# ZhuoQiuMcgill/ReinforcementLearning4MeshGeneration

Measured on AMD Instinct MI355X. Metric: env-steps/sec at N_envs=4096 per GPU, boundary() domain, 1 MI355X, higher is better.
Workload: dtype f64

## Files before the change

reinforcementlearning4meshgeneration_amd/build.py:

```python
from __future__ import annotations

import os
import shutil
import subprocess
import sys

PKG_DIR = os.path.dirname(os.path.abspath(__file__))
CSRC = os.path.join(PKG_DIR, "csrc")
LIB_NAME = "libmeshenv_hip.so"
LIB_PATH = os.path.join(PKG_DIR, LIB_NAME)
SOURCES = ["meshenv_hip.hip"]
ARCH = "gfx950"
PUBLIC_HEADERS = ["meshenv.h", "meshenv_optim.h", "meshenv_td3_actor_grad.h", "meshenv_ppo_grad.h", "meshenv_rollout.h"]

HIPCC_FLAGS = ["-O3", "-std=c++17", "-ffp-contract=off", "-fhip-fp32-correctly-rounded-divide-sqrt",
               "-fno-fast-math", "-fPIC", "-shared", f"--offload-arch={ARCH}", "-Wall", "-Wno-unused-function",
               "-mllvm", "-disable-machine-licm", "-mllvm", "-amdgpu-atomic-optimizer-strategy=None"]


def hipcc_path() -> str:
    for cand in (os.environ.get("HIPCC"), shutil.which("hipcc"), "/opt/rocm/bin/hipcc"):
        if cand and os.path.exists(cand):
            return cand
    raise RuntimeError("hipcc not found (need ROCm to build libmeshenv_hip.so)")


def needs_build() -> bool:
    if not os.path.exists(LIB_PATH):
        return True
    t = os.path.getmtime(LIB_PATH)
    deps = [os.path.join(CSRC, f) for f in sorted(os.listdir(CSRC)) if f.endswith((".h", ".hip"))]
    deps += [os.path.join(os.path.dirname(PKG_DIR), "include", h) for h in PUBLIC_HEADERS]
    return any(os.path.getmtime(d) > t for d in deps)


def build(force: bool = False, verbose: bool = False, extra_flags=()) -> str:
    if not force and not needs_build():
        return LIB_PATH
    cmd = [hipcc_path(), *HIPCC_FLAGS, *extra_flags, "-o", LIB_PATH] + [os.path.join(CSRC, s) for s in SOURCES]
    if verbose:
        print(" ".join(cmd), flush=True)
    subprocess.check_call(cmd, cwd=CSRC)
    import hashlib
    import json
    h = hashlib.sha256()
    root = os.path.dirname(PKG_DIR)
    files = sorted(os.path.join(CSRC, f) for f in os.listdir(CSRC) if f.endswith((".h", ".hip"))) + [os.path.join(root, "include", h) for h in PUBLIC_HEADERS]
    for f in files:
        h.update(os.path.relpath(f, root).encode())
        h.update(open(f, "rb").read())
# ... 7 lines not shown
```

reinforcementlearning4meshgeneration_amd/csrc/meshenv_fused.h:

```cpp
#pragma once

#include "meshenv_actor.h"
#include "meshenv_kernels.h"

namespace meshenv {

struct GroupActorArgs {
    GroupArgs g;
    ActorWeights W;
    float *actions_next;
    float *eps_out;
    unsigned long long seed, counter;
    int sample;
    int pad;
};

__host__ __device__ __forceinline__ size_t group_actor_lds_bytes(int cap)
{
    return group_lds_bytes(cap, 16) + sizeof(float) * kActorLdsFloats;
}

template <bool kDefaultParams, bool kSmall = false>
__global__ void __launch_bounds__(64 * 16)
k_step_group_actor(GroupActorArgs A)
{
    extern __shared__ double2 smem[];
    float *lds = (float *)((char *)smem + group_lds_bytes(A.g.cap, 16));
    step_group_body<16, kDefaultParams, false, kSmall>(A.g, lds);
    ActorHead hd;
    actor_request_weights(hd, A.W, threadIdx.x, true);
    __syncthreads();
    actor_forward_tile(A.W, hd, A.g.S.n_envs, blockIdx.x * kActEnvs, nullptr, nullptr, A.actions_next, A.sample, A.seed, A.counter,
                       A.eps_out, lds, threadIdx.x, 64 * 16);
}

}
```

reinforcementlearning4meshgeneration_amd/csrc/meshenv_hip.hip:

```cpp
#include "../../include/meshenv.h"
#include "../../include/meshenv_optim.h"
#include "../../include/meshenv_td3_actor_grad.h"
#include "../../include/meshenv_ppo_grad.h"
#include "../../include/meshenv_rollout.h"

#include <hip/hip_runtime.h>
#include <link.h>

#include <cmath>
#include <cstdio>
#include <cstdlib>
#include <cstring>
#include <mutex>
#include <string>
#include <vector>

#include "meshenv_actor.h"
#include "meshenv_domgen.h"
#include "meshenv_kernels.h"
#include "meshenv_quality.h"
#include "meshenv_smooth.h"
#include "meshenv_samples.h"
#include "meshenv_fused.h"
#include "meshenv_policy.h"
// ... 403 lines not shown
    constexpr int kLdsCap = 160 * 1024;
    if (lds > 64 * 1024) {
        CREATE_HIP(hipFuncSetAttribute((const void *)k_step<false, false>, hipFuncAttributeMaxDynamicSharedMemorySize, kLdsCap));
        CREATE_HIP(hipFuncSetAttribute((const void *)k_step<true, false>, hipFuncAttributeMaxDynamicSharedMemorySize, kLdsCap));
        CREATE_HIP(hipFuncSetAttribute((const void *)k_step<false, true>, hipFuncAttributeMaxDynamicSharedMemorySize, kLdsCap));
        CREATE_HIP(hipFuncSetAttribute((const void *)k_step<true, true>, hipFuncAttributeMaxDynamicSharedMemorySize, kLdsCap));
        CREATE_HIP(hipFuncSetAttribute((const void *)k_step<false, false, true>, hipFuncAttributeMaxDynamicSharedMemorySize, kLdsCap));
        CREATE_HIP(hipFuncSetAttribute((const void *)k_step<true, false, true>, hipFuncAttributeMaxDynamicSharedMemorySize, kLdsCap));
        CREATE_HIP(hipFuncSetAttribute((const void *)k_step<false, true, true>, hipFuncAttributeMaxDynamicSharedMemorySize, kLdsCap));
        CREATE_HIP(hipFuncSetAttribute((const void *)k_step<true, true, true>, hipFuncAttributeMaxDynamicSharedMemorySize, kLdsCap));
        CREATE_HIP(hipFuncSetAttribute((const void *)k_step<false, true, false, false, true>, hipFuncAttributeMaxDynamicSharedMemorySize, kLdsCap));
        CREATE_HIP(hipFuncSetAttribute((const void *)k_reset, hipFuncAttributeMaxDynamicSharedMemorySize, kLdsCap));
        CREATE_HIP(hipFuncSetAttribute((const void *)k_init_domains, hipFuncAttributeMaxDynamicSharedMemorySize, kLdsCap));
    }
    CREATE_HIP(upload_atan_state());

    {
        int n_cu = 256;
        CREATE_HIP(hipDeviceGetAttribute(&n_cu, hipDeviceAttributeMultiprocessorCount, device));
        if (n_cu <= 0) n_cu = 256;
        h->n_cu = n_cu;
        int G = 1;
        const char *force = getenv("MESHENV_GROUP");
        int want = 1;
        if (force) want = atoi(force);
        else if (n_envs <= n_cu * 16) {
            int g = 1;
            while (g * 2 <= n_envs / n_cu && g * 2 <= 16) g *= 2;
            want = g >= 8 ? g : 1;
        }
        for (int g : {16, 8})
            if (g <= want && group_lds_bytes(cap, g) <= 150 * 1024) { G = g; break; }
        if (!force && (G < 8 || n_envs > n_cu * G)) G = 1;
        if (G == 1 && want == 16 && n_envs <= n_cu * 16 && group_lds_bytes(cap, 16) > 150 * 1024) {
            std::vector<int2> pack((size_t)n_envs);
            size_t worst = 0;
            for (int w0 = 0; w0 < n_envs; w0 += 16) {
                size_t off = 0;
                for (int e = w0; e < w0 + 16 && e < n_envs; e++) {
                    const int d = env_domain_host[e];
                    const int n0 = dom_offsets_host[d + 1] - dom_offsets_host[d];
                    const int cap_e = (n0 + 15) / 16 * 16;
                    pack[(size_t)e] = make_int2((int)off, cap_e);
                    off += lds_bytes_for(cap_e);
                }
                worst = off > worst ? off : worst;
            }
            worst = (worst + 31) / 32 * 32;
            if (worst + 16 * sizeof(Handoff) <= (size_t)kLdsCap) {
                G = 16;
                h->env_lds_host.swap(pack);
                h->ho_off = (int)worst;
            }
        }
        MeshEnvParams def;
        meshenv_default_params(&def);
        h->default_params = prm.radius == def.radius && prm.max_ref_angle == def.max_ref_angle && prm.key_lambda == def.key_lambda &&
                            prm.min_degree == def.min_degree && prm.max_degree == def.max_degree &&
                            prm.same_point_eps == def.same_point_eps && prm.ray_length == def.ray_length;
        if (!h->default_params) G = 1;
        if (!h->default_params) h->env_lds_host.clear();
        h->group = G;
        h->group_lds = h->env_lds_host.empty() ? group_lds_bytes(cap, G) : (size_t)h->ho_off + 16 * sizeof(Handoff);
        {
            const char *lz = getenv("MESHENV_LAZY");
            const bool lazy = lz ? atoi(lz) != 0 : n_envs >= 8192;
            const char *lt = getenv("MESHENV_LIGHT");
// ... 718 lines not shown
    }
    return MESHENV_OK;
}

static int launch_step(MeshEnv *h, int n_steps, const float *actions_dev, float *obs_dev, double *reward_dev,
                       uint8_t *done_dev, uint8_t *complete_dev, float *terminal_obs_dev, int auto_reset)
{
    if (!h) return MESHENV_E_ARG;
    if (!actions_dev || !obs_dev || !reward_dev || !done_dev || !complete_dev) return fail_arg(h, "meshenv_step: null device pointer");
    if (n_steps <= 0) return fail_arg(h, "meshenv_rollout: n_steps must be positive");
    if (n_steps > 1 && h->reselect_pending) {
        h->err = "meshenv_rollout: the first step after meshenv_smooth must be a meshenv_step (it commits the re-selection "
                 "the candidate rebuild parked, include/meshenv.h)";
        return MESHENV_E_STATE;
    }
    MESHENV_ON_DEVICE(h);
    const size_t slot = (size_t)(h->ev_count % MESHENV_TIMING_POOL);
    const long long pos = h->timing > 0 ? (h->launch_count++ % (2LL * h->timing)) : -1;
    if (pos == 0) HIP_TRY(h, hipEventRecord(h->ev[2 * slot], h->stream));
    if (n_steps == 1 && h->group > 1 && !h->front_moved) {
        const int G = h->group;
        const dim3 grid((h->n_envs + G - 1) / G), block(64 * G);
        GroupArgs A;
        A.S = h->S;
        A.outs.obs_out = obs_dev; A.outs.reward = reward_dev; A.outs.done = done_dev; A.outs.complete = complete_dev;
        A.outs.term_obs = terminal_obs_dev;
        A.actions = actions_dev;
        A.step0 = (unsigned long long)h->steps_done;
        A.cap = h->cap;
        A.auto_reset = auto_reset;
        A.env_lds = h->env_lds;
        A.ho_off = h->ho_off;
        A.pad = 0;
        if (h->env_lds) hipLaunchKernelGGL((k_step_group<16, true, true>), grid, block, h->group_lds, h->stream, A);
        else if (h->cap <= 64 && G == 16) hipLaunchKernelGGL((k_step_group<16, true, false, true>), grid, block, h->group_lds, h->stream, A);
        else if (h->cap <= 64) hipLaunchKernelGGL((k_step_group<8, true, false, true>), grid, block, h->group_lds, h->stream, A);
        else if (G == 16) hipLaunchKernelGGL((k_step_group<16, true>), grid, block, h->group_lds, h->stream, A);
        else hipLaunchKernelGGL((k_step_group<8, true>), grid, block, h->group_lds, h->stream, A);
    } else {
        const dim3 grid(h->n_envs), block(64);
#define MESHENV_LAUNCH_STEP(MULTI, DEF)                                                                                      \
    do {                                                                                                                     \
        KStepArgs ka;                                                                                                        \
        ka.S = h->S; ka.cap = h->cap; ka.n_steps = n_steps; ka.actions = actions_dev; ka.obs_out = obs_dev;                  \
        ka.reward = reward_dev; ka.done = done_dev; ka.complete = complete_dev; ka.term_obs = terminal_obs_dev;              \
        ka.auto_reset = auto_reset; ka.step0 = (unsigned long long)h->steps_done;                                            \
        if (h->front_moved) hipLaunchKernelGGL((k_step<MULTI, DEF, true>), grid, block, h->lds, h->stream, ka);              \
        else if (DEF && !MULTI && (h->stage_bits & 2) && h->cap <= 64)                                                       \
            hipLaunchKernelGGL((k_step<false, DEF, false, DEF, DEF>), grid, block, h->lds, h->stream, ka);                   \
        else if (DEF && !MULTI && (h->stage_bits & 2))                                                                       \
            hipLaunchKernelGGL((k_step<false, DEF, false, false, DEF>), grid, block, h->lds, h->stream, ka);                 \
        else if (DEF && h->cap <= 64) hipLaunchKernelGGL((k_step<MULTI, DEF, false, DEF>), grid, block, h->lds, h->stream, ka); \
        else hipLaunchKernelGGL((k_step<MULTI, DEF>), grid, block, h->lds, h->stream, ka);                                   \
    } while (0)
        if (n_steps == 1) {
            auto_reset = (auto_reset ? 1 : 0) | h->stage_bits;
            if (h->default_params) MESHENV_LAUNCH_STEP(false, true);
            else MESHENV_LAUNCH_STEP(false, false);
        } else {
            if (h->default_params) MESHENV_LAUNCH_STEP(true, true);
            else MESHENV_LAUNCH_STEP(true, false);
        }
#undef MESHENV_LAUNCH_STEP
    }
    HIP_TRY(h, hipGetLastError());
    if (h->reselect_pending) {
        hipLaunchKernelGGL(k_apply_reselect, dim3(h->n_envs), dim3(64), 0, h->stream, h->S, h->pend, h->pend_obs, obs_dev);
        HIP_TRY(h, hipGetLastError());
        h->reselect_pending = false;
    }
    h->steps_done += (uint64_t)n_steps;
// ... 482 lines not shown
        h->err = "meshenv_step_actor: env and actor must be on the same device and stream (meshenv_set_stream / meshenv_actor_set_stream)";
        return MESHENV_E_STATE;
    }
    const bool fusable = h->group == 16 && h->default_params && !h->front_moved && !h->env_lds &&
                         h->timing == 0 && !h->reselect_pending && group_actor_lds_bytes(h->cap) <= 160 * 1024;
    if (!fusable) {
        const int rc = launch_step(h, 1, actions_dev, obs_dev, reward_dev, done_dev, complete_dev, terminal_obs_dev, auto_reset);
        if (rc != MESHENV_OK) return rc;
        const int ra = actor_launch(a, "meshenv_step_actor", h->n_envs, obs_dev, nullptr, actions_next_dev, sample, seed, counter,
                                    eps_out_dev);
        if (ra != MESHENV_OK) h->err = a->err;
        return ra;
    }
    MESHENV_ON_DEVICE(h);
    if (!h->fused_ready) {
        HIP_TRY(h, hipFuncSetAttribute((const void *)k_step_group_actor<true>, hipFuncAttributeMaxDynamicSharedMemorySize, 160 * 1024));
        HIP_TRY(h, hipFuncSetAttribute((const void *)k_step_group_actor<true, true>, hipFuncAttributeMaxDynamicSharedMemorySize, 160 * 1024));
        h->fused_ready = true;
    }
    GroupActorArgs GA;
    GA.g.S = h->S;
    GA.g.outs.obs_out = obs_dev; GA.g.outs.reward = reward_dev; GA.g.outs.done = done_dev; GA.g.outs.complete = complete_dev;
    GA.g.outs.term_obs = terminal_obs_dev;
    GA.g.actions = actions_dev;
    GA.g.step0 = (unsigned long long)h->steps_done;
    GA.g.cap = h->cap;
    GA.g.env_lds = nullptr; GA.g.ho_off = 0; GA.g.pad = 0;
    GA.g.auto_reset = auto_reset;
    GA.W = a->W;
    GA.actions_next = actions_next_dev;
    GA.eps_out = eps_out_dev;
    GA.seed = seed; GA.counter = counter;
    GA.sample = sample ? 1 : 0; GA.pad = 0;
    if (h->cap <= 64) hipLaunchKernelGGL((k_step_group_actor<true, true>), dim3((h->n_envs + 15) / 16), dim3(64 * 16), group_actor_lds_bytes(h->cap), h->stream, GA);
    else hipLaunchKernelGGL((k_step_group_actor<true>), dim3((h->n_envs + 15) / 16), dim3(64 * 16), group_actor_lds_bytes(h->cap), h->stream, GA);
    HIP_TRY(h, hipGetLastError());
    h->steps_done += 1;
    return MESHENV_OK;
}

int meshenv_extract_samples(MeshEnv *h, int which, const uint8_t *mask_dev, int n_neighbor, int n_radius, double radius, int index,
                            double quality_threshold, int64_t *count_dev, uint8_t *status_dev, const int64_t *offsets_dev,
                            double *samples_dev, double *outputs_dev, double *types_dev)
{
    if (!h || (which != 0 && which != 1) || !count_dev || !status_dev) return MESHENV_E_ARG;
    if (n_neighbor < 1 || n_neighbor > kSampMaxNeighbor || n_radius < 1 || n_radius > kSampMaxRadius || !(radius > 0) ||
        (index != 1 && index != 5))
        return fail_arg(h, "meshenv_extract_samples: n_neighbor in 1..3, n_radius in 1..4, radius > 0 and index 1 or 5 (the values of the reference's callers) are supported");
    if (offsets_dev && (!samples_dev || !outputs_dev || !types_dev))
        return fail_arg(h, "meshenv_extract_samples: offsets_dev given without the three output arrays");
    const int log_cap = h->S.prm.log_cap;
    if (log_cap <= 0) {
        h->err = "meshenv_extract_samples: handle was created with log_capacity = 0 (the mesh graph is rebuilt from the element log)";
        return MESHENV_E_STATE;
    }
    const size_t lds = samples_lds_bytes(h->cap, log_cap);
    if (lds > 160 * 1024 || h->cap + log_cap > 65535)
        return fail_arg(h, "meshenv_extract_samples: ring stride + log_capacity too large for the kernel's LDS (49 B per vertex)");
    MESHENV_ON_DEVICE(h);
    int rc = ensure_libm_tables(h);
    if (rc != MESHENV_OK) return rc;
    if (!h->samples_ready) {
        HIP_TRY(h, hipFuncSetAttribute((const void *)k_extract_samples<false>, hipFuncAttributeMaxDynamicSharedMemorySize, 160 * 1024));
        HIP_TRY(h, hipFuncSetAttribute((const void *)k_extract_samples<true>, hipFuncAttributeMaxDynamicSharedMemorySize, 160 * 1024));
        h->samples_ready = true;
    }
    SampleParams P;
    P.n_neighbor = n_neighbor; P.n_radius = n_radius; P.index = index; P.radius = radius; P.quality_threshold = quality_threshold;
// ... 1417 lines not shown
```

reinforcementlearning4meshgeneration_amd/csrc/meshenv_kernels.h:

```cpp
#pragma once

#include "meshenv_geom.h"
#include "meshenv_libm.h"
#include "meshenv_state.h"

namespace meshenv {

constexpr int kStNoReference = 1;
constexpr int kStLogOverflow = 2;
constexpr int kStRm1Bad = 4, kStRp1Bad = 8;
constexpr int kNvMeta = 8;
constexpr int kStLogHalf = 16;

#ifdef MESHENV_STAMPS
#define MESHENV_STAMP(c, k) do { if ((c).lane == 0) (c).sc->stamps[k] = __builtin_amdgcn_s_memrealtime(); } while (0)
#else
#define MESHENV_STAMP(c, k) do { } while (0)
#endif

struct Scratch {
    double2 q[4];
    double ang[4];
    double tmp[16];
    double tmp2[8];
    float robs[18];
    int ipad[2];
    unsigned long long red[6];
#ifdef MESHENV_STAMPS
    unsigned long long stamps[16];
#endif
};

struct Ctx {
    double2 *xy;
    double *key;
    int32_t *stamp;
    int32_t *id;
    double *ang_ord;
    int32_t *list;
    Scratch *sc;
    int lane, env;
    size_t base;
    int n, ref, n_elem, failed, n_new, counter, status, dom;
    double bl, area, ct, st;
    bool ring_dirty;
    bool tie = false;
    float obs;
};

__device__ __forceinline__ P2 ldp(const Ctx &c, int i)
{
    const double2 v = c.xy[i];
    return mkp(v.x, v.y);
}

__device__ __forceinline__ void wave_sync()
{
    __builtin_amdgcn_fence(__ATOMIC_ACQ_REL, "wavefront");
    __builtin_amdgcn_wave_barrier();
}

__device__ __forceinline__ int spin_until_nonzero(volatile int *w)
{
    int v = *w;
    for (int it = 0; v == 0 && it < (1 << 22); it++) {
        __builtin_amdgcn_s_sleep(1);
        v = *w;
    }
    return v;
}

__device__ __forceinline__ int wrapi(int i, int n)
{
    const unsigned a = (unsigned)i, b = (unsigned)(i + n), c = (unsigned)(i - n);
    const unsigned m = a < b ? a : b;
    return (int)(m < c ? m : c);
}

__host__ __device__ __forceinline__ size_t lds_bytes_for(int cap)
// ... 28 lines not shown
    const size_t base = (size_t)env * S.cap;
    L.s = S.scal[env];
    const int first = S.cap < 64 ? S.cap : 64;
    const double2 *gxy = S.ring_xy + base;
    const int32_t *gid = S.ring_id + base;
    const double *gkey = S.ring_key + base;
    const int32_t *gst = S.ring_stamp + base;
    const unsigned ul = (unsigned)lane;
    L.v_xy = make_double2(0, 0); L.w_xy = make_double2(0, 0);
    L.v_key = 0; L.w_key = 0;
    L.v_id = 0; L.v_st = kNotCand; L.w_id = 0; L.w_st = kNotCand;
    if (lane < first) {
        L.v_xy = gxy[ul];
        L.v_id = gid[ul];
        if (with_keys) {
            L.v_key = gkey[ul];
            L.v_st = gst[ul];
        }
    }
    const bool second = S.cap > 64 && (int)(64u + ul) < S.cap;
    if (second) {
        L.w_xy = gxy[64u + ul];
        L.w_id = gid[64u + ul];
        if (with_keys) {
            L.w_key = gkey[64u + ul];
            L.w_st = gst[64u + ul];
        }
    }
    L.obs = lane < kObsDim ? S.obs_cache[(size_t)env * kObsDim + lane] : 0.0f;
    return L;
}

__device__ __forceinline__ void load_env_commit(Ctx &c, const DevState &S, int env, const EnvLoad &L, const bool with_keys = true,
                                                const int lds_cap = 0)
{
    const int lane = lane_id();
    c.lane = lane;
    c.env = env;
    c.base = (size_t)env * S.cap;
    const EnvScalars &s = L.s;
    const int lcap = lds_cap > 0 ? lds_cap : S.cap;
    const int first = lcap < 64 ? lcap : 64;
    const double2 *gxy = S.ring_xy + c.base;
    const int32_t *gid = S.ring_id + c.base;
    const double *gkey = S.ring_key + c.base;
    const int32_t *gst = S.ring_stamp + c.base;
    const unsigned ul = (unsigned)lane;
    const bool second = lcap > 64 && (int)(64u + ul) < lcap;
    c.obs = L.obs;
    c.n = uniform_i32(s.n); c.ref = uniform_i32(s.ref); c.n_elem = uniform_i32(s.n_elem);
    c.failed = uniform_i32(s.failed); c.n_new = uniform_i32(s.n_new); c.counter = uniform_i32(s.counter);
    c.status = uniform_i32(s.status); c.dom = uniform_i32(s.dom);
    c.bl = uniform_f64(s.bl); c.area = uniform_f64(s.area); c.ct = uniform_f64(s.ct); c.st = uniform_f64(s.st);
    c.ring_dirty = false;
    if (lane < first) {
        c.xy[lane] = L.v_xy;
        c.id[lane] = L.v_id;
        if (with_keys) {
            c.key[lane] = L.v_key;
            c.stamp[lane] = L.v_st;
        }
    }
    if (second) {
        c.xy[64u + ul] = L.w_xy;
        c.id[64u + ul] = L.w_id;
        if (with_keys) {
            c.key[64u + ul] = L.w_key;
            c.stamp[64u + ul] = L.w_st;
        }
    }
    for (unsigned i = 128u + ul; i < (unsigned)c.n; i += 64u) {
        c.xy[i] = gxy[i];
        c.id[i] = gid[i];
        if (with_keys) {
            c.key[i] = gkey[i];
            c.stamp[i] = gst[i];
        }
    }
    wave_sync();
}

__device__ __forceinline__ void load_env(Ctx &c, const DevState &S, int env, const bool with_keys = true, const int lds_cap = 0)
{
    const EnvLoad L = load_env_issue(S, env, with_keys);
    load_env_commit(c, S, env, L, with_keys, lds_cap);
}

__device__ __forceinline__ void load_keys(Ctx &c, const DevState &S)
{
    const double *gkey = S.ring_key + c.base;
    const int32_t *gst = S.ring_stamp + c.base;
    for (unsigned i = (unsigned)c.lane; i < (unsigned)c.n; i += 64u) {
        c.key[i] = gkey[i];
        c.stamp[i] = gst[i];
    }
    wave_sync();
}

__device__ __forceinline__ void store_ring(const Ctx &c, const DevState &S)
{
    double2 *gxy = S.ring_xy + c.base;
    int32_t *gid = S.ring_id + c.base;
    double *gkey = S.ring_key + c.base;
    int32_t *gst = S.ring_stamp + c.base;
    for (unsigned i = (unsigned)c.lane; i < (unsigned)c.n; i += 64u) {
        gxy[i] = c.xy[i];
        gid[i] = c.id[i];
        gkey[i] = c.key[i];
        gst[i] = c.stamp[i];
    }
}

__device__ __forceinline__ void store_env(Ctx &c, const DevState &S, bool ring_elsewhere = false)
{
    wave_sync();
    if (c.ring_dirty) {
        if (!ring_elsewhere) store_ring(c, S);
        if (c.lane < kObsDim) S.obs_cache[(size_t)c.env * kObsDim + c.lane] = c.obs;
// ... 594 lines not shown
    for (int j0 = 0; j0 < total && !any_hit; j0 += 64) {
        const int j = j0 + lane;
        const bool in = j < total;
        const int i = c.list[in ? (j >> 2) : 0];
        const int nb = (j & 2) ? wrapi(i + 1, n) : wrapi(i - 1, n);
        const bool use = in && !(nb == mp0 || nb == mp1 || nb == mp2 || nb == mp3);
        const P2 ea = (j & 1) ? c0b : c0a, eb = (j & 1) ? c1b : c0b;
        const bool hit = use && is_cross(ea, eb, ldp(c, i), ldp(c, nb));
        any_hit = __ballot(hit) != 0ULL;
    }
    wave_sync();
    return any_hit;
}

__device__ __forceinline__ double quad_max_dist(int lane, P2 ref, P2 a, P2 b, P2 cpt)
{
    const P2 o = lane == 0 ? a : (lane == 1 ? b : cpt);
    const double d = dist(ref, o);
    const double d0 = lane_f64(d, 0), d1 = lane_f64(d, 1), d2 = lane_f64(d, 2);
    double m = d0 > d1 ? d0 : d1;
    return d2 > m ? d2 : m;
}


__device__ __forceinline__ void reset_from_domain(Ctx &c, const DevState &S)
{
    int half = c.status & kStLogHalf;
    if (S.prm.log_cap > 0 && c.n_elem > 0) {
        if (c.lane == 0) {
            LastEpisode le;
            le.n_elem = c.n_elem;
            le.n_new = c.n_new;
            le.flags = (c.n <= 5 ? 1 : 0) | (c.status & kStLogOverflow);
            LastEpisode *last_ep = load_cold(S).last_ep;
            le.episodes = last_ep[c.env].episodes + 1;
            last_ep[c.env] = le;
        }
        half ^= kStLogHalf;
    }
    const DomConst dc = S.dom[c.dom];
    const DevCold cold = load_cold(S);
    const int doff = uniform_i32(dc.off), n0 = uniform_i32(dc.n0);
    wave_sync();
    for (int i = c.lane; i < n0; i += 64) {
        c.xy[i] = cold.dom_xy[doff + i];
        c.id[i] = i;
        c.key[i] = cold.dom_key[doff + i];
        c.stamp[i] = cold.dom_stamp[doff + i];
    }
    c.n = n0;
    c.ref = uniform_i32(dc.ref);
    c.bl = uniform_f64(dc.bl);
    c.ct = uniform_f64(dc.ct);
    c.st = uniform_f64(dc.st);
    c.area = uniform_f64(dc.orig_area);
    c.n_elem = 0; c.failed = 0; c.n_new = 0; c.counter = 0;
    c.status = (c.ref < 0 ? kStNoReference : 0) | half;
    c.obs = c.lane < kObsDim ? cold.dom_obs[(size_t)c.dom * kObsDim + c.lane] : 0.0f;
    c.ring_dirty = true;
    wave_sync();
}

__device__ __forceinline__ void log_quad(Ctx &c, const DevState &S, int g0, int g1, int g2, int g3)
{
    const int cap = S.prm.log_cap;
    if (c.n_elem < cap) {
        if (c.lane == 0) {
            int32_t *dst = load_cold(S).log_quads + (((size_t)c.env * 2 + ((c.status >> 4) & 1)) * cap + c.n_elem) * 4;
            dst[0] = g0; dst[1] = g1; dst[2] = g2; dst[3] = g3;
        }
    } else if (cap > 0) {
        c.status |= kStLogOverflow;
    }
    c.n_elem += 1;
}

struct QuadPlan {
    int mp0, mp1, mp2, mp3, r;
    int p0, p1, p2, p3;
    int t0, t1;
    int bc0, bc1;
    VRing vr;
};

__device__ __forceinline__ QuadPlan plan_quad(bool new_vertex, int rule, int index, int n, P2 new_point)
{
    QuadPlan q;
    if (new_vertex) {
        q.mp0 = -1; q.mp1 = wrapi(index - 1, n); q.mp2 = index; q.mp3 = wrapi(index + 1, n); q.r = 2;
    } else if (rule == -1) {
        q.mp0 = wrapi(index - 1, n); q.mp1 = index; q.mp2 = wrapi(index + 1, n); q.mp3 = wrapi(index + 2, n); q.r = 1;
    } else {
        q.mp0 = wrapi(index - 2, n); q.mp1 = wrapi(index - 1, n); q.mp2 = index; q.mp3 = wrapi(index + 1, n); q.r = 2;
    }
    q.vr.is_new = new_vertex;
    q.vr.new_point = new_point;
    q.t0 = 0; q.t1 = 0;
    if (new_vertex) {
        q.vr.n = n; q.vr.lo = index; q.vr.hi = -1;
        q.p0 = wrapi(index + 1, n); q.p1 = wrapi(index - 1, n); q.p2 = wrapi(index + 2, n); q.p3 = wrapi(index - 2, n);
        q.bc0 = wrapi(index + 1, n); q.bc1 = wrapi(index - 1, n);
// ... 227 lines not shown
        mn = e2 < mn ? e2 : mn;
        mn = e3 < mn ? e3 : mn;
        e_reward = 0.0;
        if (!has_helper) {
            const double q1 = sqrt(2.0) * mn / (d13 > d02 ? d13 : d02);
            double amn = ang1 < ang0 ? ang1 : ang0, amx = ang1 > ang0 ? ang1 : ang0;
            amn = ang2 < amn ? ang2 : amn; amx = ang2 > amx ? ang2 : amx;
            amn = ang3 < amn ? ang3 : amn; amx = ang3 > amx ? ang3 : amx;
            e_reward = uniform_f64(sqrt(q1 * (amn / amx)));
        }
        bq.skip = has_helper;
        bq.half01 = uniform_f64(0.5 * e0 * e1);
        bq.half23 = uniform_f64(0.5 * e2 * e3);
        bq.q_ang0 = ang0;
        bq.q_ang2 = ang2;
        bq.ang0 = c.sc->tmp[8];
        bq.ang1 = c.sc->tmp[9];
    }
    double kk = 0.0;
    bool okk = false;
    int pos = 0;
    if (lane < 4) {
        pos = lane == 0 ? d.p0 : lane == 1 ? d.p1 : lane == 2 ? d.p2 : d.p3;
        okk = key_from_angles(prm, c.sc->tmp[2 * lane], c.sc->tmp[2 * lane + 1], kk);
    }

    wave_sync();
    if (new_vertex) {
        if (lane == 0) {
            c.xy[index] = make_double2(d.new_point.x, d.new_point.y);
            c.id[index] = kNewBit | c.n_new;
            c.stamp[index] = kNotCand;
            const int cap = prm.log_cap;
            if (c.n_new < cap) load_cold(S).log_vxy[((size_t)c.env * 2 + ((c.status >> 4) & 1)) * cap + c.n_new] = make_double2(d.new_point.x, d.new_point.y);
        }
        if (prm.log_cap > 0 && c.n_new >= prm.log_cap) c.status |= kStLogOverflow;
        c.n_new += 1;
        bq.mode = 1; bq.a = index; bq.b = 0;
    } else {
        const int lo = d.lo, hi = d.hi;
        for (int base = 0; base < n; base += 64) {
            const int i = base + lane;
            double2 vxy = make_double2(0, 0);
            double vk = 0; int vs = 0, vid = 0;
            const bool live = i < n && i != lo && i != hi;
            if (live) { vxy = c.xy[i]; vk = c.key[i]; vs = c.stamp[i]; vid = c.id[i]; }
            wave_sync();
            if (live) {
                const int j = i - (i > lo ? 1 : 0) - (i > hi ? 1 : 0);
                c.xy[j] = vxy; c.key[j] = vk; c.stamp[j] = vs; c.id[j] = vid;
            }
            wave_sync();
        }
        c.n = n - 2;
        bq.mode = 2; bq.a = d.t0; bq.b = d.t1;
    }
    wave_sync();
    {
        const unsigned long long mk = __ballot(okk);
        if (lane < 4) {
            if (okk) {
                c.key[pos] = kk;
                c.stamp[pos] = c.counter + __popcll(mk & ((2ULL << lane) - 1ULL));
            } else {
                c.stamp[pos] = kNotCand;
            }
        }
// ... 548 lines not shown
    int env, n, ref, n_elem, failed, n_new, counter, status, dom;
    int lds_off, lds_cap;
    int pad;
    double bl, area, ct, st;
    EnvCounters cnt0;
    Decision d;
};

__host__ __device__ __forceinline__ size_t group_lds_bytes(int cap, int G)
{
    return (size_t)G * (lds_bytes_for(cap) + sizeof(Handoff));
}

struct StepOuts {
    float *obs_out;
    double *reward;
    uint8_t *done;
    uint8_t *complete;
    float *term_obs;
};

struct GroupArgs {
    DevState S;
    StepOuts outs;
    const float *actions;
    unsigned long long step0;
    int cap;
    int auto_reset;
    const int2 *env_lds;
    int ho_off;
    int pad;
};

__device__ __forceinline__ StepOuts late_outs()
{
    typedef const __attribute__((address_space(4))) char *kptr;
    kptr ka = (kptr)__builtin_amdgcn_kernarg_segment_ptr();
    asm volatile("" : "+s"(ka));
    typedef const __attribute__((address_space(4))) unsigned long long *qptr;
    qptr q = (qptr)(ka + offsetof(GroupArgs, outs));
    static_assert(sizeof(StepOuts) == 5 * sizeof(unsigned long long), "StepOuts is five pointers");
    StepOuts o;
    o.obs_out = (float *)q[0];
    o.reward = (double *)q[1];
    o.done = (uint8_t *)q[2];
    o.complete = (uint8_t *)q[3];
    o.term_obs = (float *)q[4];
    return o;
}

__device__ __forceinline__ DevState late_state(const DevState &S)
{
    typedef const __attribute__((address_space(4))) unsigned long long *qptr;
    qptr q = (qptr)__builtin_amdgcn_kernarg_segment_ptr();
    asm volatile("" : "+s"(q));
    constexpr unsigned kWords = offsetof(DevState, prm) / 8;
    static_assert(offsetof(DevState, prm) % 8 == 0, "whole quadwords before prm");
    union { DevState s; unsigned long long w[sizeof(DevState) / 8]; } u;
    u.s = S;
#pragma unroll
    for (unsigned i = 0; i < kWords; i++) u.w[i] = q[i];
    return u.s;
}

__device__ __forceinline__ void finish_and_store(Ctx &c, const DevState &S_in, const Decision &d, const EnvCounters &cnt0,
                                                 int n_before, int auto_reset, unsigned long long step0,
                                                 volatile int *helper_done = nullptr, float *actor_row = nullptr,
                                                 const bool cnt_late = false)
{
    const StepResult r = env_finish(c, S_in.prm, d);
    const int env = c.env;
    const DevState S = late_state(S_in);
    const StepOuts o = late_outs();
    float *__restrict__ obs_out = o.obs_out;
    double *__restrict__ reward = o.reward;
    uint8_t *__restrict__ done = o.done;
    uint8_t *__restrict__ complete = o.complete;
    float *__restrict__ term_obs = o.term_obs;
    const bool has_helper = helper_done != nullptr;
    if (c.lane == 0) {
        if (!has_helper) reward[env] = r.reward;
        done[env] = (uint8_t)r.done;
        complete[env] = (uint8_t)r.complete;
    }
    if (r.done) {
        if (term_obs && c.lane < kObsDim) term_obs[(size_t)env * kObsDim + c.lane] = c.obs;
        if (auto_reset) {
            if (has_helper) {
                spin_until_nonzero(helper_done);
                wave_sync();
            }
            reset_from_domain(c, S);
        }
    }
    if (c.lane < kObsDim) obs_out[(size_t)env * kObsDim + c.lane] = c.obs;
    if (actor_row && c.lane < kObsDim) actor_row[(c.lane & 3) * 8 + (c.lane >> 2)] = c.obs;
    if (S.msg && c.lane < 21 && !(has_helper && c.lane == 18)) {
        const float v = c.lane < kObsDim ? c.obs : (c.lane == 18 ? (float)r.reward : (c.lane == 19 ? (float)r.done : (float)r.complete));
        S.msg[(size_t)env * 21 + c.lane] = v;
    }
    store_env(c, S, has_helper && !r.done);
    if ((r.valid || (r.done && auto_reset)) && c.lane == 0) {
        EnvCounters k = cnt_late ? S.cnt[env] : cnt0;
        k.sum_n += (unsigned long long)n_before * (step0 + 1ULL - k.last_change);
        k.last_change = step0 + 1ULL;
        if (r.valid) { k.valid += 1ULL; k.sum_n_valid += (unsigned long long)n_before; }
        S.cnt[env] = k;
    }
}

template <int G, bool kDefaultParams, bool kRagged = false, bool kSmall = false>
__device__ __forceinline__ void step_group_body(const GroupArgs &A, float *actor_in = nullptr)
{
    const int tid = (int)threadIdx.x;
    extern __shared__ double2 smem[];
    DevState S = A.S;
    const int cap = A.cap, auto_reset = A.auto_reset;
    if (kSmall) __builtin_assume(cap <= 64 && S.cap <= 64 && cap > 0 && S.cap > 0);
    const float *__restrict__ actions = A.actions;
    if (kDefaultParams) apply_default_params(S.prm);
    const int wave = uniform_i32(tid >> 6);
    const size_t env_bytes = lds_bytes_for(cap);
    Handoff *ho = (Handoff *)((char *)smem + (kRagged ? (size_t)A.ho_off : (size_t)G * env_bytes));
    const int env = blockIdx.x * G + wave;
    const bool active = env < S.n_envs;
    int pending = 0;
#ifdef MESHENV_STAMPS
    const unsigned long long dbg_t0 = __builtin_amdgcn_s_memrealtime();
#endif
    if (active) {
        Ctx c;
        int my_off = (int)((size_t)wave * env_bytes), my_cap = cap;
        if (kRagged) {
            const int2 e = A.env_lds[env];
            my_off = uniform_i32(e.x);
            my_cap = uniform_i32(e.y);
        }
        carve_lds(c, (char *)smem + my_off, my_cap);
        const float *a = actions + (size_t)env * 3;
        const float a0 = a[0], a1 = a[1], a2 = a[2];
        EnvCounters cnt0;
        cnt0.last_change = 0; cnt0.valid = 0; cnt0.sum_n = 0; cnt0.sum_n_valid = 0;
        constexpr bool kCntLate = true;
        load_env(c, S, env, true, kRagged ? my_cap : 0);
        if (kSmall) __builtin_assume(c.n <= 64 && c.n >= 0);
        const int n_before = c.n;
        Decision d = env_check(c, S, a0, a1, a2, false, false, 0.0, 0.0, 0.5, true);
        if (!d.ok) {
            finish_and_store(c, S, d, cnt0, n_before, auto_reset, A.step0, nullptr, actor_in ? actor_in + wave * 132 : nullptr, kCntLate);
        } else {
            pending = 1;
            if (c.lane == 0) {
                Handoff &h = ho[wave];
                h.env = env; h.n = c.n; h.ref = c.ref; h.n_elem = c.n_elem; h.failed = c.failed; h.n_new = c.n_new;
                h.counter = c.counter; h.status = c.status; h.dom = c.dom;
                if (kRagged) { h.lds_off = my_off; h.lds_cap = my_cap; }
                h.bl = c.bl; h.area = c.area; h.ct = c.ct; h.st = c.st;
                h.d = d;
                h.upd_done = 0;
                h.helper_done = 0;
            }
        }
    }
    if ((tid & 63) == 0) {
        ho[wave].valid = pending;
        ho[wave].simd = (int)__builtin_amdgcn_s_getreg((4 << 0) | (4 << 6) | (1 << 11));
    }
#ifdef MESHENV_STAMPS
    const unsigned long long dbg_t1 = __builtin_amdgcn_s_memrealtime();
#endif
    __syncthreads();
#ifdef MESHENV_STAMPS
    const unsigned long long dbg_t2 = __builtin_amdgcn_s_memrealtime();
    if (active && (tid & 63) == 0) {
        unsigned long long *o = S.dbg + (size_t)env * 16;
        o[0] = dbg_t0; o[1] = dbg_t1; o[2] = dbg_t2; o[3] = (unsigned long long)pending; o[4] = 0; o[5] = 0;
#ifdef MESHENV_DBG_P1SET
        {
            Ctx cs;
            carve_lds(cs, (char *)smem + (kRagged ? A.env_lds[env].x : (int)((size_t)wave * env_bytes)), kRagged ? A.env_lds[env].y : cap);
            o[4] = cs.sc->stamps[MESHENV_DBG_P1SET ? 4 : 1];
            o[5] = cs.sc->stamps[MESHENV_DBG_P1SET ? 5 : 2];
// ... 22 lines not shown
#ifdef MESHENV_NO_HELPER
    const bool helpers = false;
#else
    const bool helpers = balanced && G >= 4 && 2 * m <= G && m <= 8;
#endif
    if (balanced && G >= 4) {
        const int r = __popc(mine & ((1u << wave) - 1u));
        const int j = r * 4 + my_simd;
        int k = j < m ? j : -1;
        if (helpers && j >= m) {
            const unsigned long long t_lo = G >= 16 ? 0x1111300011000010ULL : 0x1111210011000010ULL;
            const unsigned long long t_hi = 0x2222321133001220ULL;
            const unsigned hcw = (unsigned)(((m <= 4 ? t_lo : t_hi) >> (16 * ((m - 1) & 3))) & 0xffffULL);
            const int mains_here = (m + 3 - my_simd) >> 2;
            const int t = r - mains_here;
            const int here = (int)((hcw >> (4 * my_simd)) & 15u);
            const int below = my_simd == 0 ? 0 : (int)((hcw & 15u) + (my_simd > 1 ? ((hcw >> 4) & 15u) : 0u) + (my_simd > 2 ? ((hcw >> 8) & 15u) : 0u));
            if (t >= 0 && t < here) k = below + t;
        }
        if (k >= 0) {
            unsigned rest = vmask;
            for (int t = 0; t < k; t++) rest &= rest - 1u;
            const int which = __ffs((int)rest) - 1;
            if (j < m) src = which;
            else hsrc = which;
        }
    } else if (vmask & (1u << wave)) {
        src = wave;
    }
    if (src < 0 && hsrc < 0) return;

    if (hsrc >= 0) {
        Ctx c;
        Handoff &h = ho[hsrc];
        if (kRagged) carve_lds(c, (char *)smem + uniform_i32(h.lds_off), uniform_i32(h.lds_cap));
        else carve_lds(c, (char *)smem + (size_t)hsrc * env_bytes, cap);
        c.lane = tid & 63;
        Decision d = h.d;
        d.index = uniform_i32(d.index); d.new_vertex = uniform_i32(d.new_vertex);
        d.t0 = uniform_i32(d.t0); d.t1 = uniform_i32(d.t1);
        const int henv = uniform_i32(h.env);
        const double rew = reward_on_helper(c, S, d, uniform_i32(h.n), uniform_i32(h.dom), &h.upd_done);
        wave_sync();
        if (c.n > 5) {
            c.env = henv;
            c.base = (size_t)henv * S.cap;
            store_ring(c, late_state(S));
        }
        if (c.lane == 0) {
            *(volatile int *)&h.helper_done = 1;
            const StepOuts o = late_outs();
            o.reward[henv] = rew;
            if (S.msg) S.msg[(size_t)henv * 21 + 18] = (float)rew;
        }
        return;
    }

    Ctx c;
    Handoff &h = ho[src];
    if (kRagged) carve_lds(c, (char *)smem + uniform_i32(h.lds_off), uniform_i32(h.lds_cap));
    else carve_lds(c, (char *)smem + (size_t)src * env_bytes, cap);
    c.lane = tid & 63;
    c.env = uniform_i32(h.env);
    c.base = (size_t)c.env * S.cap;
    c.n = uniform_i32(h.n); c.ref = uniform_i32(h.ref); c.n_elem = uniform_i32(h.n_elem); c.failed = uniform_i32(h.failed);
    if (kSmall) __builtin_assume(c.n <= 64 && c.n >= 0);
    c.n_new = uniform_i32(h.n_new); c.counter = uniform_i32(h.counter); c.status = uniform_i32(h.status); c.dom = uniform_i32(h.dom);
    c.bl = uniform_f64(h.bl); c.area = uniform_f64(h.area); c.ct = uniform_f64(h.ct); c.st = uniform_f64(h.st);
    c.ring_dirty = false;
    c.obs = 0.0f;
    Decision d = h.d;
    d.index = uniform_i32(d.index); d.new_vertex = uniform_i32(d.new_vertex);
    d.mp0 = uniform_i32(d.mp0); d.mp1 = uniform_i32(d.mp1); d.mp2 = uniform_i32(d.mp2); d.mp3 = uniform_i32(d.mp3);
    d.p0 = uniform_i32(d.p0); d.p1 = uniform_i32(d.p1); d.p2 = uniform_i32(d.p2); d.p3 = uniform_i32(d.p3);
    d.t0 = uniform_i32(d.t0); d.t1 = uniform_i32(d.t1); d.lo = uniform_i32(d.lo); d.hi = uniform_i32(d.hi);
    d.ok = 1;
    const EnvCounters cnt0 = S.cnt[c.env];
    const int n_before = c.n;
    env_apply(c, S, d, helpers ? &h.upd_done : nullptr);
#ifdef MESHENV_STAMPS
    const unsigned long long dbg_t8 = __builtin_amdgcn_s_memrealtime();
#endif
    finish_and_store(c, S, d, cnt0, n_before, auto_reset, A.step0, helpers ? &h.helper_done : nullptr,
                     actor_in ? actor_in + src * 132 : nullptr);
#ifdef MESHENV_STAMPS
    if (c.lane == 0) {
        const unsigned long long t_end = __builtin_amdgcn_s_memrealtime();
        unsigned long long *o = S.dbg + (size_t)c.env * 16;
        o[6] = c.sc->stamps[6]; o[7] = dbg_t2; o[8] = dbg_t8;
        for (int k = 9; k <= 14; k++) o[k] = c.sc->stamps[k];
        o[15] = t_end;
        if (active) {
            unsigned long long *w = S.dbg + (size_t)env * 16;
            w[4] = t_end; w[5] = (unsigned long long)(src + 1);
        }
    }
#endif
}


template <int G, bool kDefaultParams, bool kRagged = false, bool kSmall = false>
__global__ void __launch_bounds__(64 * G)
k_step_group(GroupArgs A)
{
    step_group_body<G, kDefaultParams, kRagged, kSmall>(A);
}

}
```

reinforcementlearning4meshgeneration_amd/csrc/meshenv_state.h:

```cpp
#pragma once

#include <hip/hip_runtime.h>
#include <stdint.h>

namespace meshenv {

constexpr int kObsDim = 18;
constexpr int kNotCand = INT32_MIN;

struct alignas(64) EnvScalars {
    int32_t n;
    int32_t ref;
    int32_t n_elem;
    int32_t n_new;
    int32_t counter;
    int32_t dom;
    int32_t failed;
    int32_t status;
    double bl;
    double area;
    double ct, st;
};

struct alignas(32) EnvCounters {
// ... 37 lines not shown
};

struct DevCold {
    const double2 *dom_xy;
    double *dom_key;
    int32_t *dom_stamp;
    float *dom_obs;
    int32_t *log_quads;
    double2 *log_vxy;
    LastEpisode *last_ep;
    int64_t pad;
};

struct DevState {
    int n_domains;
    DomConst *dom;
    const DevCold *cold;
    int n_envs;
    int cap;
    double2 *ring_xy;
    int32_t *ring_id;
    double *ring_key;
    int32_t *ring_stamp;
    EnvScalars *scal;
    EnvCounters *cnt;
    float *obs_cache;
    float *msg;
#ifdef MESHENV_STAMPS
    unsigned long long *dbg;
#endif
    Params prm;
};

__device__ __forceinline__ DevCold load_cold(const DevState &S)
{
    const DevCold *p = S.cold;
    asm volatile("" : "+s"(p));
    return *p;
}

}
```

Measured before the change: 294.9 million.

## Preload hot kernel arguments into SGPRs and mark pointers as global address space

Moves the most frequently used pointers and sizes (ring buffers, scalars, actions, n_envs, cap) into leading scalar kernel parameters and enables kernarg preloading of 16 SGPRs, so the grouped step kernels start without waiting on kernarg loads. Late-read arguments such as step0 and the outputs are now read from the kernarg segment at the point of use, shifted by the preloaded block's size. Pointers are cast to the global address space so the compiler can emit global rather than flat memory instructions, and a range assumption on the ring size is added for small capacities. It also lets a forced group size fall back to ragged LDS packing. The risks are ABI and offset mismatches in the kernarg layout and higher SGPR pressure.

```diff
diff --git a/reinforcementlearning4meshgeneration_amd/build.py b/reinforcementlearning4meshgeneration_amd/build.py
--- a/reinforcementlearning4meshgeneration_amd/build.py
+++ b/reinforcementlearning4meshgeneration_amd/build.py
@@ -15,7 +15,8 @@
 
 HIPCC_FLAGS = ["-O3", "-std=c++17", "-ffp-contract=off", "-fhip-fp32-correctly-rounded-divide-sqrt",
                "-fno-fast-math", "-fPIC", "-shared", f"--offload-arch={ARCH}", "-Wall", "-Wno-unused-function",
-               "-mllvm", "-disable-machine-licm", "-mllvm", "-amdgpu-atomic-optimizer-strategy=None"]
+               "-mllvm", "-disable-machine-licm", "-mllvm", "-amdgpu-atomic-optimizer-strategy=None",
+               "-mllvm", "-amdgpu-kernarg-preload-count=16"]
 
 
 def hipcc_path() -> str:
diff --git a/reinforcementlearning4meshgeneration_amd/csrc/meshenv_fused.h b/reinforcementlearning4meshgeneration_amd/csrc/meshenv_fused.h
--- a/reinforcementlearning4meshgeneration_amd/csrc/meshenv_fused.h
+++ b/reinforcementlearning4meshgeneration_amd/csrc/meshenv_fused.h
@@ -15,6 +15,8 @@
     int pad;
 };
 
+static_assert(alignof(GroupActorArgs) == 8, "follows the leading arguments (EntryArgs) without a gap, as GroupArgs does");
+
 __host__ __device__ __forceinline__ size_t group_actor_lds_bytes(int cap)
 {
     return group_lds_bytes(cap, 16) + sizeof(float) * kActorLdsFloats;
@@ -22,11 +24,13 @@
 
 template <bool kDefaultParams, bool kSmall = false>
 __global__ void __launch_bounds__(64 * 16)
-k_step_group_actor(GroupActorArgs A)
+k_step_group_actor(MESHENV_ENTRY_PARAMS GroupActorArgs A)
 {
+    EntryArgs E;
+    MESHENV_ENTRY_PACK(E);
     extern __shared__ double2 smem[];
     float *lds = (float *)((char *)smem + group_lds_bytes(A.g.cap, 16));
-    step_group_body<16, kDefaultParams, false, kSmall>(A.g, lds);
+    step_group_body<16, kDefaultParams, false, kSmall>(E, A.g, lds);
     ActorHead hd;
     actor_request_weights(hd, A.W, threadIdx.x, true);
     __syncthreads();
diff --git a/reinforcementlearning4meshgeneration_amd/csrc/meshenv_hip.hip b/reinforcementlearning4meshgeneration_amd/csrc/meshenv_hip.hip
--- a/reinforcementlearning4meshgeneration_amd/csrc/meshenv_hip.hip
+++ b/reinforcementlearning4meshgeneration_amd/csrc/meshenv_hip.hip
@@ -459,7 +459,7 @@
         for (int g : {16, 8})
             if (g <= want && group_lds_bytes(cap, g) <= 150 * 1024) { G = g; break; }
         if (!force && (G < 8 || n_envs > n_cu * G)) G = 1;
-        if (G == 1 && want == 16 && n_envs <= n_cu * 16 && group_lds_bytes(cap, 16) > 150 * 1024) {
+        if ((G == 1 || (force && G < 16)) && want == 16 && n_envs <= n_cu * 16 && group_lds_bytes(cap, 16) > 150 * 1024) {
             std::vector<int2> pack((size_t)n_envs);
             size_t worst = 0;
             for (int w0 = 0; w0 < n_envs; w0 += 16) {
@@ -1244,11 +1244,11 @@
         A.env_lds = h->env_lds;
         A.ho_off = h->ho_off;
         A.pad = 0;
-        if (h->env_lds) hipLaunchKernelGGL((k_step_group<16, true, true>), grid, block, h->group_lds, h->stream, A);
-        else if (h->cap <= 64 && G == 16) hipLaunchKernelGGL((k_step_group<16, true, false, true>), grid, block, h->group_lds, h->stream, A);
-        else if (h->cap <= 64) hipLaunchKernelGGL((k_step_group<8, true, false, true>), grid, block, h->group_lds, h->stream, A);
-        else if (G == 16) hipLaunchKernelGGL((k_step_group<16, true>), grid, block, h->group_lds, h->stream, A);
-        else hipLaunchKernelGGL((k_step_group<8, true>), grid, block, h->group_lds, h->stream, A);
+        if (h->env_lds) hipLaunchKernelGGL((k_step_group<16, true, true>), grid, block, h->group_lds, h->stream, MESHENV_ENTRY_LAUNCH(A) A);
+        else if (h->cap <= 64 && G == 16) hipLaunchKernelGGL((k_step_group<16, true, false, true>), grid, block, h->group_lds, h->stream, MESHENV_ENTRY_LAUNCH(A) A);
+        else if (h->cap <= 64) hipLaunchKernelGGL((k_step_group<8, true, false, true>), grid, block, h->group_lds, h->stream, MESHENV_ENTRY_LAUNCH(A) A);
+        else if (G == 16) hipLaunchKernelGGL((k_step_group<16, true>), grid, block, h->group_lds, h->stream, MESHENV_ENTRY_LAUNCH(A) A);
+        else hipLaunchKernelGGL((k_step_group<8, true>), grid, block, h->group_lds, h->stream, MESHENV_ENTRY_LAUNCH(A) A);
     } else {
         const dim3 grid(h->n_envs), block(64);
 #define MESHENV_LAUNCH_STEP(MULTI, DEF)                                                                                      \
@@ -1797,8 +1797,8 @@
     GA.eps_out = eps_out_dev;
     GA.seed = seed; GA.counter = counter;
     GA.sample = sample ? 1 : 0; GA.pad = 0;
-    if (h->cap <= 64) hipLaunchKernelGGL((k_step_group_actor<true, true>), dim3((h->n_envs + 15) / 16), dim3(64 * 16), group_actor_lds_bytes(h->cap), h->stream, GA);
-    else hipLaunchKernelGGL((k_step_group_actor<true>), dim3((h->n_envs + 15) / 16), dim3(64 * 16), group_actor_lds_bytes(h->cap), h->stream, GA);
+    if (h->cap <= 64) hipLaunchKernelGGL((k_step_group_actor<true, true>), dim3((h->n_envs + 15) / 16), dim3(64 * 16), group_actor_lds_bytes(h->cap), h->stream, MESHENV_ENTRY_LAUNCH(GA.g) GA);
+    else hipLaunchKernelGGL((k_step_group_actor<true>), dim3((h->n_envs + 15) / 16), dim3(64 * 16), group_actor_lds_bytes(h->cap), h->stream, MESHENV_ENTRY_LAUNCH(GA.g) GA);
     HIP_TRY(h, hipGetLastError());
     h->steps_done += 1;
     return MESHENV_OK;
diff --git a/reinforcementlearning4meshgeneration_amd/csrc/meshenv_kernels.h b/reinforcementlearning4meshgeneration_amd/csrc/meshenv_kernels.h
--- a/reinforcementlearning4meshgeneration_amd/csrc/meshenv_kernels.h
+++ b/reinforcementlearning4meshgeneration_amd/csrc/meshenv_kernels.h
@@ -45,6 +45,7 @@
     double bl, area, ct, st;
     bool ring_dirty;
     bool tie = false;
+    bool cold_global = false;
     float obs;
 };
 
@@ -139,7 +140,7 @@
 }
 
 __device__ __forceinline__ void load_env_commit(Ctx &c, const DevState &S, int env, const EnvLoad &L, const bool with_keys = true,
-                                                const int lds_cap = 0)
+                                                const int lds_cap = 0, const bool small = false)
 {
     const int lane = lane_id();
     c.lane = lane;
@@ -160,6 +161,7 @@
     c.status = uniform_i32(s.status); c.dom = uniform_i32(s.dom);
     c.bl = uniform_f64(s.bl); c.area = uniform_f64(s.area); c.ct = uniform_f64(s.ct); c.st = uniform_f64(s.st);
     c.ring_dirty = false;
+    if (small) __builtin_assume(c.n <= 64 && c.n >= 0);
     if (lane < first) {
         c.xy[lane] = L.v_xy;
         c.id[lane] = L.v_id;
@@ -187,10 +189,11 @@
     wave_sync();
 }
 
-__device__ __forceinline__ void load_env(Ctx &c, const DevState &S, int env, const bool with_keys = true, const int lds_cap = 0)
+__device__ __forceinline__ void load_env(Ctx &c, const DevState &S, int env, const bool with_keys = true, const int lds_cap = 0,
+                                         const bool small = false)
 {
     const EnvLoad L = load_env_issue(S, env, with_keys);
-    load_env_commit(c, S, env, L, with_keys, lds_cap);
+    load_env_commit(c, S, env, L, with_keys, lds_cap, small);
 }
 
 __device__ __forceinline__ void load_keys(Ctx &c, const DevState &S)
@@ -851,14 +854,14 @@
             le.n_elem = c.n_elem;
             le.n_new = c.n_new;
             le.flags = (c.n <= 5 ? 1 : 0) | (c.status & kStLogOverflow);
-            LastEpisode *last_ep = load_cold(S).last_ep;
+            LastEpisode *last_ep = load_cold(S, c.cold_global).last_ep;
             le.episodes = last_ep[c.env].episodes + 1;
             last_ep[c.env] = le;
         }
         half ^= kStLogHalf;
     }
     const DomConst dc = S.dom[c.dom];
-    const DevCold cold = load_cold(S);
+    const DevCold cold = load_cold(S, c.cold_global);
     const int doff = uniform_i32(dc.off), n0 = uniform_i32(dc.n0);
     wave_sync();
     for (int i = c.lane; i < n0; i += 64) {
@@ -885,7 +888,7 @@
     const int cap = S.prm.log_cap;
     if (c.n_elem < cap) {
         if (c.lane == 0) {
-            int32_t *dst = load_cold(S).log_quads + (((size_t)c.env * 2 + ((c.status >> 4) & 1)) * cap + c.n_elem) * 4;
+            int32_t *dst = load_cold(S, c.cold_global).log_quads + (((size_t)c.env * 2 + ((c.status >> 4) & 1)) * cap + c.n_elem) * 4;
             dst[0] = g0; dst[1] = g1; dst[2] = g2; dst[3] = g3;
         }
     } else if (cap > 0) {
@@ -1179,7 +1182,7 @@
             c.id[index] = kNewBit | c.n_new;
             c.stamp[index] = kNotCand;
             const int cap = prm.log_cap;
-            if (c.n_new < cap) load_cold(S).log_vxy[((size_t)c.env * 2 + ((c.status >> 4) & 1)) * cap + c.n_new] = make_double2(d.new_point.x, d.new_point.y);
+            if (c.n_new < cap) load_cold(S, c.cold_global).log_vxy[((size_t)c.env * 2 + ((c.status >> 4) & 1)) * cap + c.n_new] = make_double2(d.new_point.x, d.new_point.y);
         }
         if (prm.log_cap > 0 && c.n_new >= prm.log_cap) c.status |= kStLogOverflow;
         c.n_new += 1;
@@ -1794,21 +1797,47 @@
     int pad;
 };
 
+struct EntryArgs {
+    double2 *ring_xy;
+    int32_t *ring_id;
+    double *ring_key;
+    int32_t *ring_stamp;
+    EnvScalars *scal;
+    const float *actions;
+    int n_envs, cap;
+};
+constexpr unsigned kEntryBytes = sizeof(EntryArgs);
+static_assert(sizeof(EntryArgs) == 14 * 4, "fourteen dwords: the preload limit");
+#define MESHENV_ENTRY_PARAMS double2 *e_ring_xy, int32_t *e_ring_id, double *e_ring_key, int32_t *e_ring_stamp, EnvScalars *e_scal, \
+                             const float *e_actions, int e_n_envs, int e_cap,
+#define MESHENV_ENTRY_PACK(E)                                                                                            \
+    E.ring_xy = e_ring_xy; E.ring_id = e_ring_id; E.ring_key = e_ring_key; E.ring_stamp = e_ring_stamp; E.scal = e_scal; \
+    E.actions = e_actions; E.n_envs = e_n_envs; E.cap = e_cap
+#define MESHENV_ENTRY_LAUNCH(A) (A).S.ring_xy, (A).S.ring_id, (A).S.ring_key, (A).S.ring_stamp, (A).S.scal, (A).actions, (A).S.n_envs, (A).S.cap,
+
 __device__ __forceinline__ StepOuts late_outs()
 {
     typedef const __attribute__((address_space(4))) char *kptr;
     kptr ka = (kptr)__builtin_amdgcn_kernarg_segment_ptr();
     asm volatile("" : "+s"(ka));
     typedef const __attribute__((address_space(4))) unsigned long long *qptr;
-    qptr q = (qptr)(ka + offsetof(GroupArgs, outs));
+    qptr q = (qptr)(ka + kEntryBytes + offsetof(GroupArgs, outs));
     static_assert(sizeof(StepOuts) == 5 * sizeof(unsigned long long), "StepOuts is five pointers");
     StepOuts o;
-    o.obs_out = (float *)q[0];
-    o.reward = (double *)q[1];
-    o.done = (uint8_t *)q[2];
-    o.complete = (uint8_t *)q[3];
-    o.term_obs = (float *)q[4];
+    o.obs_out = as_global((float *)q[0]);
+    o.reward = as_global((double *)q[1]);
+    o.done = as_global((uint8_t *)q[2]);
+    o.complete = as_global((uint8_t *)q[3]);
+    o.term_obs = as_global((float *)q[4]);
     return o;
+}
+
+__device__ __forceinline__ unsigned long long late_step0()
+{
+    typedef const __attribute__((address_space(4))) char *kptr;
+    kptr ka = (kptr)__builtin_amdgcn_kernarg_segment_ptr();
+    asm volatile("" : "+s"(ka));
+    return *(const __attribute__((address_space(4))) unsigned long long *)(ka + kEntryBytes + offsetof(GroupArgs, step0));
 }
 
 __device__ __forceinline__ DevState late_state(const DevState &S)
@@ -1816,17 +1845,27 @@
     typedef const __attribute__((address_space(4))) unsigned long long *qptr;
     qptr q = (qptr)__builtin_amdgcn_kernarg_segment_ptr();
     asm volatile("" : "+s"(q));
+    static_assert(kEntryBytes % 8 == 0 && alignof(GroupArgs) == 8, "the argument block follows the leading arguments without a gap");
+    q += kEntryBytes / 8;
     constexpr unsigned kWords = offsetof(DevState, prm) / 8;
     static_assert(offsetof(DevState, prm) % 8 == 0, "whole quadwords before prm");
     union { DevState s; unsigned long long w[sizeof(DevState) / 8]; } u;
     u.s = S;
 #pragma unroll
     for (unsigned i = 0; i < kWords; i++) u.w[i] = q[i];
+    u.s.dom = as_global(u.s.dom); u.s.cold = as_global(u.s.cold);
+    u.s.ring_xy = as_global(u.s.ring_xy); u.s.ring_id = as_global(u.s.ring_id);
+    u.s.ring_key = as_global(u.s.ring_key); u.s.ring_stamp = as_global(u.s.ring_stamp);
+    u.s.scal = as_global(u.s.scal); u.s.cnt = as_global(u.s.cnt);
+    u.s.obs_cache = as_global(u.s.obs_cache); u.s.msg = as_global(u.s.msg);
+#ifdef MESHENV_STAMPS
+    u.s.dbg = as_global(u.s.dbg);
+#endif
     return u.s;
 }
 
 __device__ __forceinline__ void finish_and_store(Ctx &c, const DevState &S_in, const Decision &d, const EnvCounters &cnt0,
-                                                 int n_before, int auto_reset, unsigned long long step0,
+                                                 int n_before, int auto_reset,
                                                  volatile int *helper_done = nullptr, float *actor_row = nullptr,
                                                  const bool cnt_late = false)
 {
@@ -1864,6 +1903,7 @@
     store_env(c, S, has_helper && !r.done);
     if ((r.valid || (r.done && auto_reset)) && c.lane == 0) {
         EnvCounters k = cnt_late ? S.cnt[env] : cnt0;
+        const unsigned long long step0 = late_step0();
         k.sum_n += (unsigned long long)n_before * (step0 + 1ULL - k.last_change);
         k.last_change = step0 + 1ULL;
         if (r.valid) { k.valid += 1ULL; k.sum_n_valid += (unsigned long long)n_before; }
@@ -1872,14 +1912,17 @@
 }
 
 template <int G, bool kDefaultParams, bool kRagged = false, bool kSmall = false>
-__device__ __forceinline__ void step_group_body(const GroupArgs &A, float *actor_in = nullptr)
+__device__ __forceinline__ void step_group_body(const EntryArgs &E, const GroupArgs &A, float *actor_in = nullptr)
 {
     const int tid = (int)threadIdx.x;
     extern __shared__ double2 smem[];
     DevState S = A.S;
-    const int cap = A.cap, auto_reset = A.auto_reset;
+    S.ring_xy = E.ring_xy; S.ring_id = E.ring_id; S.ring_key = E.ring_key; S.ring_stamp = E.ring_stamp; S.scal = E.scal;
+    S.n_envs = E.n_envs; S.cap = E.cap;
+    const float *__restrict__ actions = E.actions;
+    const int cap = E.cap;
+    const int auto_reset = A.auto_reset;
     if (kSmall) __builtin_assume(cap <= 64 && S.cap <= 64 && cap > 0 && S.cap > 0);
-    const float *__restrict__ actions = A.actions;
     if (kDefaultParams) apply_default_params(S.prm);
     const int wave = uniform_i32(tid >> 6);
     const size_t env_bytes = lds_bytes_for(cap);
@@ -1892,6 +1935,7 @@
 #endif
     if (active) {
         Ctx c;
+        c.cold_global = true;
         int my_off = (int)((size_t)wave * env_bytes), my_cap = cap;
         if (kRagged) {
             const int2 e = A.env_lds[env];
@@ -1904,12 +1948,14 @@
         EnvCounters cnt0;
         cnt0.last_change = 0; cnt0.valid = 0; cnt0.sum_n = 0; cnt0.sum_n_valid = 0;
         constexpr bool kCntLate = true;
-        load_env(c, S, env, true, kRagged ? my_cap : 0);
+        EnvLoad L = load_env_issue(S, env, true);
+        asm("" : "+s"(L.s.n) : "s"(a0), "s"(a1), "s"(a2));
+        load_env_commit(c, S, env, L, true, kRagged ? my_cap : 0, kSmall);
         if (kSmall) __builtin_assume(c.n <= 64 && c.n >= 0);
         const int n_before = c.n;
         Decision d = env_check(c, S, a0, a1, a2, false, false, 0.0, 0.0, 0.5, true);
         if (!d.ok) {
-            finish_and_store(c, S, d, cnt0, n_before, auto_reset, A.step0, nullptr, actor_in ? actor_in + wave * 132 : nullptr, kCntLate);
+            finish_and_store(c, S, d, cnt0, n_before, auto_reset, nullptr, actor_in ? actor_in + wave * 132 : nullptr, kCntLate);
         } else {
             pending = 1;
             if (c.lane == 0) {
@@ -1998,6 +2044,7 @@
 
     if (hsrc >= 0) {
         Ctx c;
+        c.cold_global = true;
         Handoff &h = ho[hsrc];
         if (kRagged) carve_lds(c, (char *)smem + uniform_i32(h.lds_off), uniform_i32(h.lds_cap));
         else carve_lds(c, (char *)smem + (size_t)hsrc * env_bytes, cap);
@@ -2008,21 +2055,23 @@
         const int henv = uniform_i32(h.env);
         const double rew = reward_on_helper(c, S, d, uniform_i32(h.n), uniform_i32(h.dom), &h.upd_done);
         wave_sync();
+        const DevState SL = late_state(S);
         if (c.n > 5) {
             c.env = henv;
             c.base = (size_t)henv * S.cap;
-            store_ring(c, late_state(S));
+            store_ring(c, SL);
         }
         if (c.lane == 0) {
             *(volatile int *)&h.helper_done = 1;
             const StepOuts o = late_outs();
             o.reward[henv] = rew;
-            if (S.msg) S.msg[(size_t)henv * 21 + 18] = (float)rew;
+            if (SL.msg) SL.msg[(size_t)henv * 21 + 18] = (float)rew;
         }
         return;
     }
 
     Ctx c;
+    c.cold_global = true;
     Handoff &h = ho[src];
     if (kRagged) carve_lds(c, (char *)smem + uniform_i32(h.lds_off), uniform_i32(h.lds_cap));
     else carve_lds(c, (char *)smem + (size_t)src * env_bytes, cap);
@@ -2047,7 +2096,7 @@
 #ifdef MESHENV_STAMPS
     const unsigned long long dbg_t8 = __builtin_amdgcn_s_memrealtime();
 #endif
-    finish_and_store(c, S, d, cnt0, n_before, auto_reset, A.step0, helpers ? &h.helper_done : nullptr,
+    finish_and_store(c, S, d, cnt0, n_before, auto_reset, helpers ? &h.helper_done : nullptr,
                      actor_in ? actor_in + src * 132 : nullptr);
 #ifdef MESHENV_STAMPS
     if (c.lane == 0) {
@@ -2067,9 +2116,11 @@
 
 template <int G, bool kDefaultParams, bool kRagged = false, bool kSmall = false>
 __global__ void __launch_bounds__(64 * G)
-k_step_group(GroupArgs A)
-{
-    step_group_body<G, kDefaultParams, kRagged, kSmall>(A);
-}
-
-}
+k_step_group(MESHENV_ENTRY_PARAMS GroupArgs A)
+{
+    EntryArgs E;
+    MESHENV_ENTRY_PACK(E);
+    step_group_body<G, kDefaultParams, kRagged, kSmall>(E, A);
+}
+
+}
diff --git a/reinforcementlearning4meshgeneration_amd/csrc/meshenv_state.h b/reinforcementlearning4meshgeneration_amd/csrc/meshenv_state.h
--- a/reinforcementlearning4meshgeneration_amd/csrc/meshenv_state.h
+++ b/reinforcementlearning4meshgeneration_amd/csrc/meshenv_state.h
@@ -93,11 +93,22 @@
     Params prm;
 };
 
-__device__ __forceinline__ DevCold load_cold(const DevState &S)
+template <class T>
+__device__ __forceinline__ T *as_global(T *p)
+{
+    return (T *)(__attribute__((address_space(1))) T *)(unsigned long long)p;
+}
+
+__device__ __forceinline__ DevCold load_cold(const DevState &S, const bool global = false)
 {
     const DevCold *p = S.cold;
     asm volatile("" : "+s"(p));
-    return *p;
+    if (!global) return *p;
+    DevCold c = *as_global(p);
+    c.dom_xy = as_global(c.dom_xy); c.dom_key = as_global(c.dom_key); c.dom_stamp = as_global(c.dom_stamp);
+    c.dom_obs = as_global(c.dom_obs); c.log_quads = as_global(c.log_quads); c.log_vxy = as_global(c.log_vxy);
+    c.last_ep = as_global(c.last_ep);
+    return c;
 }
 
 }
```

Result: faster. 302.5 million, median of 6 (+2.6%).
